# timoklein/alphazero-gym

Measured on AMD Instinct MI355X. Metric: MCTS sims/sec (whole node), Pendulum-v1 4096 trees n_sims=200, 1/2/4/8 GPU, higher is better.
Workload: dtype f32; 1 GPU; config C: Pendulum-v1 A0C, 4096 trees/GPU x 200 sims, 2x256 ELU policy/value MLP, c_uct=0.05 c_pw=1 kappa=0.5; trees_per_gpu=4096, n_sims=200, parallelism=1 GPU

## Files before the change

### alphazero_gym_amd/csrc/mlp.cuh

```cuda
#pragma once
#include "records.h"


typedef int i32x4 __attribute__((ext_vector_type(4)));


__device__ __forceinline__ f32x4 expm1f4_nonpos(f32x4 xc) {
    const f32x4 magic = {12582912.0f, 12582912.0f, 12582912.0f, 12582912.0f};
    const f32x4 l2e = {1.44269504088896341f, 1.44269504088896341f, 1.44269504088896341f, 1.44269504088896341f};
    const f32x4 ln2h = {0.693145751953125f, 0.693145751953125f, 0.693145751953125f, 0.693145751953125f};
    const f32x4 ln2l = {1.42860682030941723212e-6f, 1.42860682030941723212e-6f, 1.42860682030941723212e-6f, 1.42860682030941723212e-6f};
    const f32x4 kb = __builtin_elementwise_fma(xc, l2e, magic);
    const f32x4 kf = kb - magic;
    f32x4 r = __builtin_elementwise_fma(-kf, ln2h, xc);
    r = __builtin_elementwise_fma(-kf, ln2l, r);
    f32x4 p = {1.98412698412698413e-4f, 1.98412698412698413e-4f, 1.98412698412698413e-4f, 1.98412698412698413e-4f};
    const f32x4 c5 = {1.38888888888888894e-3f, 1.38888888888888894e-3f, 1.38888888888888894e-3f, 1.38888888888888894e-3f};
    const f32x4 c4 = {8.33333333333333322e-3f, 8.33333333333333322e-3f, 8.33333333333333322e-3f, 8.33333333333333322e-3f};
    const f32x4 c3 = {4.16666666666666644e-2f, 4.16666666666666644e-2f, 4.16666666666666644e-2f, 4.16666666666666644e-2f};
    const f32x4 c2 = {1.66666666666666657e-1f, 1.66666666666666657e-1f, 1.66666666666666657e-1f, 1.66666666666666657e-1f};
    const f32x4 half = {0.5f, 0.5f, 0.5f, 0.5f}, one = {1.0f, 1.0f, 1.0f, 1.0f};
    p = __builtin_elementwise_fma(p, r, c5);
    p = __builtin_elementwise_fma(p, r, c4);
    p = __builtin_elementwise_fma(p, r, c3);
    p = __builtin_elementwise_fma(p, r, c2);
    p = __builtin_elementwise_fma(p, r, half);
    f32x4 em1 = __builtin_elementwise_fma(p * r, r, r);
    const i32x4 scb = (((i32x4)kb) << 23) + 0x3F800000;
    const f32x4 sc = (f32x4)scb;
    return __builtin_elementwise_fma(sc, em1, sc - one);
}

template <bool RARE = true>
__device__ __forceinline__ f32x4 act4(int act, f32x4 v) {
    f32x4 pos;
    asm("v_max_f32 %0, 0, %1" : "=v"(pos.x) : "v"(v.x)); asm("v_max_f32 %0, 0, %1" : "=v"(pos.y) : "v"(v.y));
    asm("v_max_f32 %0, 0, %1" : "=v"(pos.z) : "v"(v.z)); asm("v_max_f32 %0, 0, %1" : "=v"(pos.w) : "v"(v.w));
    if (act == AZG_ACT_ELU) {
        f32x4 neg;
        neg.x = __builtin_amdgcn_fmed3f(v.x, -87.0f, 0.0f); neg.y = __builtin_amdgcn_fmed3f(v.y, -87.0f, 0.0f);
        neg.z = __builtin_amdgcn_fmed3f(v.z, -87.0f, 0.0f); neg.w = __builtin_amdgcn_fmed3f(v.w, -87.0f, 0.0f);
        return pos + expm1f4_nonpos(neg);
    }
    if (!RARE || act == AZG_ACT_RELU) return pos;
    f32x4 r;
    r.x = azg_activation(act, v.x); r.y = azg_activation(act, v.y); r.z = azg_activation(act, v.z); r.w = azg_activation(act, v.w);
    return r;
}

__device__ __forceinline__ f32x4 mfma4(f32x4 a, f32x4 b, f32x4 acc) {
    acc = __builtin_amdgcn_mfma_f32_16x16x4f32(a.x, b.x, acc, 0, 0, 0);
    acc = __builtin_amdgcn_mfma_f32_16x16x4f32(a.y, b.y, acc, 0, 0, 0);
    acc = __builtin_amdgcn_mfma_f32_16x16x4f32(a.z, b.z, acc, 0, 0, 0);
// ... 89 lines not shown
            } else {
#pragma unroll
                for (int i = 0; i < NT0; ++i) a0[i] = act4<false>(AZG_ACT_RELU, a0[i]);
            }
#pragma unroll
            for (int i = 0; i < NT0; ++i) actA[((wave - NW / 2) * NT0 + i) * 64 + lane] = a0[i];
            if (lane == 0) __hip_atomic_fetch_add(l0_flag, 1, __ATOMIC_RELEASE, __HIP_MEMORY_SCOPE_WORKGROUP);
        }
        const int want = (NW / 2) * step;
        while (__hip_atomic_load(l0_flag, __ATOMIC_ACQUIRE, __HIP_MEMORY_SCOPE_WORKGROUP) < want) __builtin_amdgcn_s_sleep(1);
    } else {
#pragma unroll
    for (int g = 0; g < NG; ++g) {
        float b;
        if constexpr (NT == 16) b = obsT[(lane >> 4) * (16 * NG) + g * 16 + (lane & 15)];
        else b = (lane & 15) < NT ? obsT[(lane >> 4) * (NT * NG) + g * NT + (lane & 15)] : 0.0f;
        float b2 = 0.0f;
        if constexpr (IN8) {
            if constexpr (NT == 16) b2 = obsT[(4 + (lane >> 4)) * (16 * NG) + g * 16 + (lane & 15)];
            else b2 = (lane & 15) < NT ? obsT[(4 + (lane >> 4)) * (NT * NG) + g * NT + (lane & 15)] : 0.0f;
        }
#pragma unroll
        for (int i = 0; i < NTW; ++i) {
            f32x4 a0;
            if constexpr (HP <= 256) {
                a0 = __builtin_amdgcn_mfma_f32_16x16x4f32(wr.w0[i], b, wr.b0[i], 0, 0, 0);
                if constexpr (IN8) { if (P.in8) a0 = __builtin_amdgcn_mfma_f32_16x16x4f32(wr.w0b[i], b2, a0, 0, 0, 0); }
            } else {
                const int nt = wave * NTW + i;
                a0 = __builtin_amdgcn_mfma_f32_16x16x4f32(P.W0[wofs + nt * 64 + lane], b, net_ptr(P.b0, wofs)[nt * 64 + lane], 0, 0, 0);
                if constexpr (IN8) { if (P.in8) a0 = __builtin_amdgcn_mfma_f32_16x16x4f32(P.W0b[wofs + nt * 64 + lane], b2, a0, 0, 0, 0); }
            }
            if constexpr (NREG == 0) h[g][i] = act4<true>(P.act, a0);
            else h[g][i] = a0;
        }
    }
    if constexpr (NREG > 0) {
        if (P.act == AZG_ACT_ELU) {
#pragma unroll
            for (int g = 0; g < NG; ++g)
#pragma unroll
                for (int i = 0; i < NTW; ++i) h[g][i] = act4<false>(AZG_ACT_ELU, h[g][i]);
        } else {
#pragma unroll
            for (int g = 0; g < NG; ++g)
#pragma unroll
                for (int i = 0; i < NTW; ++i) h[g][i] = act4<false>(AZG_ACT_RELU, h[g][i]);
        }
    }
    }
    if constexpr (NREG == 0) { if (P.layernorm) layer_norm_wg<HP>(P, 0, h[0], s_ln, wave, lane, wofs); }
    f32x4* buf = actA;
    f32x4* other = actB;
    if (NREG > 0) {
#pragma unroll
        for (int l = 0; l < NREG; ++l) {
            if (!(SPLIT && l == 0)) {
#pragma unroll
                for (int g = 0; g < NG; ++g)
#pragma unroll
                    for (int i = 0; i < NTW; ++i) buf[g * ABUF + (wave * NTW + i) * 64 + lane] = h[g][i];
                __syncthreads();
            }
            STAMP_M(m1, 4, 5);
            f32x4 acc[NG][NTW];
            f32x4 bcur[NG], bnext[NG];
#pragma unroll
            for (int g = 0; g < NG; ++g) {
#pragma unroll
                for (int i = 0; i < NTW; ++i) acc[g][i] = wr.b[l][i];
                bcur[g] = buf[g * ABUF + lane];
            }
#pragma unroll
            for (int s4 = 0; s4 < S4; ++s4) {
#pragma unroll
                for (int g = 0; g < NG; ++g) {
                    bnext[g] = bcur[g];
                    if (s4 + 1 < S4) bnext[g] = buf[g * ABUF + (s4 + 1) * 64 + lane];
                }
                __builtin_amdgcn_sched_barrier(0);
#pragma unroll
                for (int i = 0; i < NTW; ++i)
#pragma unroll
                    for (int g = 0; g < NG; ++g) acc[g][i] = __builtin_amdgcn_mfma_f32_16x16x4f32(wr.w[l][i][s4].x, bcur[g].x, acc[g][i], 0, 0, 0);
#pragma unroll
                for (int i = 0; i < NTW; ++i)
#pragma unroll
                    for (int g = 0; g < NG; ++g) acc[g][i] = __builtin_amdgcn_mfma_f32_16x16x4f32(wr.w[l][i][s4].y, bcur[g].y, acc[g][i], 0, 0, 0);
#pragma unroll
                for (int i = 0; i < NTW; ++i)
#pragma unroll
                    for (int g = 0; g < NG; ++g) acc[g][i] = __builtin_amdgcn_mfma_f32_16x16x4f32(wr.w[l][i][s4].z, bcur[g].z, acc[g][i], 0, 0, 0);
#pragma unroll
                for (int i = 0; i < NTW; ++i)
#pragma unroll
                    for (int g = 0; g < NG; ++g) acc[g][i] = __builtin_amdgcn_mfma_f32_16x16x4f32(wr.w[l][i][s4].w, bcur[g].w, acc[g][i], 0, 0, 0);
#pragma unroll
                for (int g = 0; g < NG; ++g) bcur[g] = bnext[g];
            }
            STAMP_M(m2, 5, 6);
            if (P.act == AZG_ACT_ELU) {
#pragma unroll
                for (int g = 0; g < NG; ++g)
#pragma unroll
                    for (int i = 0; i < NTW; ++i) h[g][i] = act4<false>(AZG_ACT_ELU, acc[g][i]);
            } else {
#pragma unroll
                for (int g = 0; g < NG; ++g)
#pragma unroll
                    for (int i = 0; i < NTW; ++i) h[g][i] = act4<false>(AZG_ACT_RELU, acc[g][i]);
            }
            STAMP_M(m2b, 6, -1);
            if (l == 0) { STAMP_M_ADD(4, m0, m1); }
            STAMP_M_ADD(5, m1, m2);
            STAMP_M_ADD(6, m2, m2b);
            f32x4* t = buf; buf = other; other = t;
        }
    } else {
        for (int l = 1; l < P.n_hidden; ++l) {
#pragma unroll
            for (int i = 0; i < NTW; ++i) buf[(wave * NTW + i) * 64 + lane] = h[0][i];
            __syncthreads();
            const f32x4* W = net_ptr(P.Wl[l - 1], wofs);
            const f32x4* bb = net_ptr(P.bl[l - 1], wofs);
            constexpr int TG = NTW < 4 ? NTW : 4;
#pragma unroll
            for (int tg = 0; tg < NTW; tg += TG) {
                f32x4 acc[TG];
#pragma unroll
                for (int i = 0; i < TG; ++i) acc[i] = bb[(wave * NTW + tg + i) * 64 + lane];
#pragma unroll 2
                for (int s4 = 0; s4 < S4; ++s4) {
                    f32x4 b = buf[s4 * 64 + lane];
                    f32x4 a[TG];
#pragma unroll
                    for (int i = 0; i < TG; ++i) a[i] = W[((wave * NTW + tg + i) * S4 + s4) * 64 + lane];
#pragma unroll
                    for (int i = 0; i < TG; ++i) acc[i] = __builtin_amdgcn_mfma_f32_16x16x4f32(a[i].x, b.x, acc[i], 0, 0, 0);
#pragma unroll
                    for (int i = 0; i < TG; ++i) acc[i] = __builtin_amdgcn_mfma_f32_16x16x4f32(a[i].y, b.y, acc[i], 0, 0, 0);
#pragma unroll
                    for (int i = 0; i < TG; ++i) acc[i] = __builtin_amdgcn_mfma_f32_16x16x4f32(a[i].z, b.z, acc[i], 0, 0, 0);
#pragma unroll
                    for (int i = 0; i < TG; ++i) acc[i] = __builtin_amdgcn_mfma_f32_16x16x4f32(a[i].w, b.w, acc[i], 0, 0, 0);
                }
#pragma unroll
                for (int i = 0; i < TG; ++i) h[0][tg + i] = act4<NREG == 0>(P.act, acc[i]);
            }
            if (P.layernorm) layer_norm_wg<HP>(P, l, h[0], s_ln, wave, lane, wofs);
            f32x4* t = buf; buf = other; other = t;
        }
    }
    {
        constexpr int NSUB = HP <= 256 ? 8 / NW : NTW / 4;
        constexpr int KS = 4 * NTW / NSUB;
        f32x4 acc[NG][NSUB];
#pragma unroll
        for (int g = 0; g < NG; ++g)
#pragma unroll
            for (int sc = 0; sc < NSUB; ++sc) acc[g][sc] = f32x4{0.0f, 0.0f, 0.0f, 0.0f};
#pragma unroll
        for (int j = 0; j < KS; ++j) {
#pragma unroll
            for (int sc = 0; sc < NSUB; ++sc) {
                const int ks = sc * KS + j, ti = ks >> 2, cmp = ks & 3;
                const f32x4 a = (NREG > 0) ? wr.wh[ti] : net_ptr(P.Whead, wofs)[(wave * NTW + ti) * 64 + lane];
#pragma unroll
                for (int g = 0; g < NG; ++g) acc[g][sc] = __builtin_amdgcn_mfma_f32_16x16x4f32(a[cmp], h[g][ti][cmp], acc[g][sc], 0, 0, 0);
            }
        }
#pragma unroll
        for (int g = 0; g < NG; ++g)
#pragma unroll
            for (int sc = 0; sc < NSUB; ++sc)
                if (PSTR == 64 || lane < 16) parts[(g * NCH + wave * NSUB + sc) * PSTR + lane] = acc[g][sc];
    }
    __syncthreads();
}

template <int NCH, int PSTR = 64>
__device__ __forceinline__ float head_output(const f32x4* parts, const float* s_bhead, int tl, int o) {
    float total = s_bhead[o];
    const int idx = (o >> 2) * 16 + tl;
#pragma unroll
    for (int w = 0; w < NCH; ++w) {
        f32x4 pv = parts[w * PSTR + idx];
        float p = (o & 3) == 0 ? pv.x : ((o & 3) == 1 ? pv.y : ((o & 3) == 2 ? pv.z : pv.w));
        total = total + p;
    }
    return total;
}

template <int NCH, int PSTR = 64>
__device__ __forceinline__ f32x4 head_output4(const f32x4* parts, const float* s_bhead, int tl) {
    f32x4 total = {s_bhead[0], s_bhead[1], s_bhead[2], s_bhead[3]};
#pragma unroll
    for (int w = 0; w < NCH; ++w) {
        const f32x4 pv = parts[w * PSTR + tl];
        total.x = total.x + pv.x; total.y = total.y + pv.y; total.z = total.z + pv.z; total.w = total.w + pv.w;
    }
    return total;
}

#define GMM_MAXC 5
template <int NCH, int PSTR = 64>
__device__ __forceinline__ void gmm_params(const f32x4* parts, const float* s_bhead, int tl, int C, float ls_min, float ls_max, float* d) {
    float mx = head_output<NCH, PSTR>(parts, s_bhead, tl, 1 + 2 * C);
#pragma unroll
    for (int c = 1; c < GMM_MAXC; ++c)
        if (c < C) { float v = head_output<NCH, PSTR>(parts, s_bhead, tl, 1 + 2 * C + c); mx = v > mx ? v : mx; }
    float ex[GMM_MAXC], sum = 0.0f, cum = 0.0f;
#pragma unroll
    for (int c = 0; c < GMM_MAXC; ++c) {
        ex[c] = 0.0f;
        if (c < C) { ex[c] = azg_expf(head_output<NCH, PSTR>(parts, s_bhead, tl, 1 + 2 * C + c) - mx); sum = sum + ex[c]; }
    }
#pragma unroll
    for (int c = 0; c < GMM_MAXC; ++c) {
        d[c] = 0.0f; d[GMM_MAXC + c] = 0.0f; d[2 * GMM_MAXC + c] = 2.0f;
        if (c < C) {
            float ls = head_output<NCH, PSTR>(parts, s_bhead, tl, 1 + C + c);
            ls = ls < ls_min ? ls_min : (ls > ls_max ? ls_max : ls);
            d[c] = head_output<NCH, PSTR>(parts, s_bhead, tl, 1 + c);
            d[GMM_MAXC + c] = azg_expf(ls);
            cum = cum + ex[c] / sum;
            d[2 * GMM_MAXC + c] = cum;
        }
    }
}

__device__ __forceinline__ void gmm_pick(const float* d, int C, unsigned long long seed, unsigned gtree, unsigned search, unsigned k,
                                         float* mu, float* sg) {
    azg_u32x4 b = azg_draw(seed, gtree, search, k, AZG_STREAM_PW);
    float u = azg_u01(b.v[2]);
    float m = 0.0f, s = 0.0f;
    bool found = false;
#pragma unroll
    for (int i = 0; i < GMM_MAXC; ++i) {
        bool last = (i == C - 1);
        if (i < C && !found && (u < d[2 * GMM_MAXC + i] || last)) { m = d[i]; s = d[GMM_MAXC + i]; found = true; }
    }
    *mu = m;
// ... 3 lines not shown
```

### alphazero_gym_amd/csrc/search_kernel.cuh

```cuda
#pragma once
#include "records.h"
#include "env.cuh"
#include "mlp.cuh"
#include "tree.cuh"
#include "tree_phases.cuh"
#include "results.cuh"
#ifndef AZG_DEFER
#define AZG_DEFER 1
#endif

struct LdsLayout {
    size_t act_off;
    size_t tree_off;
    size_t per_tree;
    size_t state_off;
    size_t total;
};
__host__ __device__ inline LdsLayout lds_layout(int tab_n, int n_sims, int HP, int NG, int nbuf, int R, bool cont, int tlds, int lds_state = 0, int NT = 16) {
    LdsLayout L;
    L.act_off = ((size_t)tab_n * 8 + (size_t)(n_sims + 2) * 2 + 15) / 16 * 16;
    L.tree_off = L.act_off + (size_t)nbuf * NG * HP * 64;
    L.per_tree = (size_t)R * 16 + (cont ? (size_t)POOL_UNITS(R) * (tlds == TS_LDS9 ? 8 : 4) : (size_t)R * 4);
    L.per_tree = (L.per_tree + 15) / 16 * 16;
    L.state_off = 0;
// ... 64 lines not shown
        constexpr int S4 = HP / 16;
#pragma unroll
        for (int l = 0; l < NREG; ++l) {
#pragma unroll
            for (int i = 0; i < NTW; ++i) {
                wr.b[l][i] = net_ptr(P.bl[l], wofs)[(wave * NTW + i) * 64 + lane];
#pragma unroll
                for (int s4 = 0; s4 < S4; ++s4) wr.w[l][i][s4] = net_ptr(P.Wl[l], wofs)[((wave * NTW + i) * S4 + s4) * 64 + lane];
            }
        }
#pragma unroll
        for (int i = 0; i < NTW; ++i) wr.wh[i] = net_ptr(P.Whead, wofs)[(wave * NTW + i) * 64 + lane];
    }

    struct Ctx {
        int sub, tl, tree; bool has_tree, live; unsigned gtree; size_t tb;
        Cold* cold; double* edge_W; float* action; TreeStore<TLDS> ts; const f32x4* my_parts;
    };
    auto make_ctx = [&](int t) {
        Ctx c;
        const int w = t >> 6, ln = t & 63;
        c.sub = ln & 15;
        c.has_tree = w < NWALK && (ln >> 4) < TPV;
        c.tl = c.has_tree ? w * TPV + (ln >> 4) : 0;
        c.tree = tree0 + c.tl;
        c.live = c.has_tree && c.tl < n_live;
        c.gtree = (unsigned)(P.tree_base + c.tree);
        c.tb = (size_t)(c.live ? c.tree : 0) * P.R;
        c.cold = P.cold + c.tb;
        c.edge_W = P.edge_W + c.tb;
        c.action = P.action + c.tb;
        if constexpr (TLDS != TS_GLOBAL) {
            char* base = (char*)s_dyn + L.tree_off + L.per_tree * c.tl;
            c.ts.hot = (Rec*)base;
            c.ts.pool = (typename TreeStore<TLDS>::PoolId*)(base + (size_t)P.R * 16);
            c.ts.prior = (float*)(base + (size_t)P.R * 16);
            c.ts.state = L.state_off ? (double*)(base + L.state_off) : nullptr;
        } else {
            c.ts.hot = (Rec*)(P.hot + c.tb);
            c.ts.child = P.child + c.tb * P.Kp;
            c.ts.prior = P.prior + c.tb;
        }
        c.my_parts = s_parts + (c.tl / NT) * NCH * PSTR;
        return c;
    };
    Ctx cx = make_ctx(tid);

#ifdef AZG_STAMPS
    unsigned long long st_acc[16] = {0, 0, 0, 0, 0, 0, 0, 0, 0, 0, 0, 0, 0, 0, 0, 0};
#endif
    TreeState st = {};
    st.need_eval = false;
    BDeferred bdef = {};
    if (cx.has_tree) tree_init_root<ENV, TLDS, TPW, IN8>(P, st, cx.ts, cx.cold, cx.edge_W, cx.action, cx.tree, cx.live, cx.sub, cx.tl, cx.gtree, s_obsT);
    __syncthreads();

    constexpr bool MULTI = !CONT;
    static_assert(!(LEAN && MULTI), "discrete 8-wave shapes: extend the LEAN packing first");
    int my_sim = -1;
    for (int sim = -1; sim < P.n_sims; ++sim) {
        STAMP2(t_a, 0, -1);
        __syncthreads();
        if constexpr (MULTI) { if (*(volatile int*)&s_done >= n_live) break; }
        STAMP2(t_b, 0, 1);
        if constexpr (DEFER) {
            STAMP2(t_b2a, 12, -1);
            if (cx.live) tree_phase_b2<ENV, TLDS, SPEC>(P, st, cx.ts, cx.cold, cx.edge_W, cx.action, bdef, cx.sub, cx.gtree, s_pw);
            bdef.pending = false;
            STAMP2(t_b2b, 12, -1);
#ifdef AZG_STAMP_ONLY
            STAMP_ADD(12, t_b2a, t_b2b);
#endif
        }
        unsigned pk0 = 0, pk1 = 0, pk2 = 0, pk3 = 0;
        int tid_o = tid;
        if constexpr (LEAN) {
            pk0 = (unsigned)st.nrec | ((unsigned)st.leaf << 16);
            pk1 = (unsigned)st.path_D | ((unsigned)st.kbase << 16);
            pk2 = (unsigned)(st.my_depth + 1) | ((unsigned)st.pid << 16);
            pk3 = (unsigned)st.ptop | ((unsigned)st.need_eval << 16) | ((unsigned)st.resume << 20);
            asm volatile("" : "+v"(pk0), "+v"(pk1), "+v"(pk2), "+v"(pk3));
        }
#ifdef AZG_STAMPS
        mlp_forward<HP, NREG, NW, NG, PSTR, WR, NT, IN8, DEFER>(P, wr, s_obsT, s_actA, s_actB, s_parts, s_ln, wave, lane, st_acc, &s_l0, sim + 2, wofs);
#else
        mlp_forward<HP, NREG, NW, NG, PSTR, WR, NT, IN8, DEFER>(P, wr, s_obsT, s_actA, s_actB, s_parts, s_ln, wave, lane, &s_l0, sim + 2, wofs);
#endif
        STAMP2(t_c, 1, 2);
        if constexpr (LEAN) {
            asm volatile("" : "+v"(pk0), "+v"(pk1), "+v"(pk2), "+v"(pk3), "+v"(tid_o));
            st.nrec = (int)(pk0 & 0xffffu); st.leaf = (int)(pk0 >> 16);
            st.path_D = (int)(pk1 & 0xffffu); st.kbase = (int)(pk1 >> 16);
            st.my_depth = (int)(pk2 & 0xffffu) - 1; st.pid = (int)(pk2 >> 16);
            st.ptop = (int)(pk3 & 0xffffu); st.need_eval = ((pk3 >> 16) & 1u) != 0; st.resume = (int)(pk3 >> 20);
            cx = make_ctx(tid_o);
            st.pr = 0.0; st.pW = 0.0;
            if (cx.live && (MULTI ? my_sim : sim) >= 0 && st.my_depth >= 1) {
                st.pr = CONT ? cx.cold[st.pid].r : discrete_env_reward(Spec<SPEC, ENV>::env(P));
                st.pW = cx.edge_W[st.pid];
            }
        }
        if constexpr (!MULTI) {
            if (cx.live) tree_phase_a<ENV, TLDS, GMM, NCH, PSTR, !CONT, SPEC>(P, st, cx.ts, cx.cold, cx.edge_W, cx.action, cx.tb, sim, cx.sub, cx.tl % NT, cx.gtree, cx.my_parts, s_bhead, s_sqrt STAMP_ARG, s_pw);
            if (sim == P.n_sims - 1) break;
            if constexpr (DEFER) { if (sim < 0 && cx.live) eps_prepare(P, st, cx.gtree, cx.sub); }
            tree_fence();
            STAMP2(t_d, 2, 3);
            st.need_eval = false;
            if (cx.live) tree_phase_b<ENV, TLDS, GMM, TPW, unsigned short, !LEAN, !CONT, SPEC, IN8, DEFER>(P, st, cx.ts, cx.cold, cx.edge_W, cx.action, cx.tb, cx.sub, cx.tl, cx.gtree, s_sqrt, s_pw, s_obsT STAMP_ARG, &bdef);
            tree_fence();
            STAMP2(t_e, 3, -1);
            STAMP_ADD(2, t_c, t_d);
            STAMP_ADD(3, t_d, t_e);
        } else {
            bool run = cx.live && my_sim < P.n_sims;
            int k = 0;
            while (run) {
                STAMP2(t_c2, 2, -1);
                tree_phase_a<ENV, TLDS, GMM, NCH, PSTR, !CONT, SPEC>(P, st, cx.ts, cx.cold, cx.edge_W, cx.action, cx.tb, my_sim, cx.sub, cx.tl % NT, cx.gtree, cx.my_parts, s_bhead, s_sqrt STAMP_ARG, s_pw);
                tree_fence();
                STAMP2(t_d, 2, 3);
                st.need_eval = false;
                if (my_sim == P.n_sims - 1) {
                    my_sim = P.n_sims;
                    if (cx.sub == 0) atomicAdd(&s_done, 1);
                    run = false;
                } else {
                    my_sim += 1;
                    tree_phase_b<ENV, TLDS, GMM, TPW, unsigned short, !LEAN, !CONT, SPEC, IN8>(P, st, cx.ts, cx.cold, cx.edge_W, cx.action, cx.tb, cx.sub, cx.tl, cx.gtree, s_sqrt, s_pw, s_obsT STAMP_ARG);
                    tree_fence();
                    k += 1;
                    if (st.need_eval || k >= P.trace_cap) run = false;
                }
                STAMP2(t_e, 3, -1);
                STAMP_ADD(2, t_c2, t_d);
                STAMP_ADD(3, t_d, t_e);
            }
        }
        STAMP_ADD(0, t_a, t_b);
        STAMP_ADD(1, t_b, t_c);
    }
    const int nrec = st.nrec;
    const int sub = cx.sub, tree = cx.tree;
    const bool live = cx.live;
    const size_t tb = cx.tb;
    const TreeStore<TLDS>& ts = cx.ts;
#ifdef AZG_STAMPS
    if (lane == 0) for (int i = 0; i < 16; ++i) P.stamps[((size_t)blockIdx.x * NW + wave) * 16 + i] = st_acc[i];
#endif
    if (live) results_for_tree<CONT, TLDS>(P, ts, cx.cold, cx.action, tb, tree, sub);
    if (live) {
        if (sub == 0) P.n_rec[tree] = nrec;
        if constexpr (TLDS != TS_GLOBAL) {
            if (P.publish) {
                RecL* gh = P.hot + tb;
                for (int j = sub; j < nrec; j += 16) {
                    Rec h = ts.hot[j];
                    RecL o;
                    o.Q = h.Q; o.edge_n = h.edge_n; o.node_n = h.node_n; o.parent = (short)h.parent; o.n_child = h.n_child;
                    o.first = CONT ? 0 : h.first; o.flags = h.flags; o.pad = 0;
                    gh[j] = o;
                    if (CONT) {
// ... 10 lines not shown
```

### alphazero_gym_amd/csrc/tree.cuh

```cuda
#pragma once
#include "records.h"

__device__ __forceinline__ void tree_fence() { __builtin_amdgcn_fence(__ATOMIC_ACQ_REL, "wavefront"); }

__device__ __forceinline__ double tree_div(double n, double d) {
    double r = __builtin_amdgcn_rcp(d);
    double e = __builtin_fma(-d, r, 1.0);
    r = __builtin_fma(r, e, r);
    e = __builtin_fma(-d, r, 1.0);
    r = __builtin_fma(r, e, r);
    double q = n * r;
    double rem = __builtin_fma(-d, q, n);
    return __builtin_fma(rem, r, q);
}


template <int CTRL>
__device__ __forceinline__ int dpp_i32(int v) { return __builtin_amdgcn_update_dpp(0, v, CTRL, 0xf, 0xf, false); }
template <int CTRL>
__device__ __forceinline__ double dpp_f64(double v) {
    unsigned long long u = azg_d2u(v);
    unsigned lo = (unsigned)dpp_i32<CTRL>((int)(unsigned)u), hi = (unsigned)dpp_i32<CTRL>((int)(unsigned)(u >> 32));
    return azg_u2d(((unsigned long long)hi << 32) | lo);
}
template <int CTRL>
__device__ __forceinline__ float dpp_f32(float v) { return __builtin_bit_cast(float, dpp_i32<CTRL>(__builtin_bit_cast(int, v))); }
#define DPP_QUAD_BCAST1 0x55
#define DPP_QUAD_XOR1 0xB1
#define DPP_QUAD_XOR2 0x4E
#define DPP_ROW_ROR4 0x124
#define DPP_ROW_ROR8 0x128
#define DPP_ROW_ROR15 0x12F

__device__ __forceinline__ double rowmax16(double u, bool valid) {
    double m = valid ? u : -__builtin_huge_val();
    double o;
    o = dpp_f64<DPP_QUAD_XOR1>(m); m = o > m ? o : m;
    o = dpp_f64<DPP_QUAD_XOR2>(m); m = o > m ? o : m;
    o = dpp_f64<DPP_ROW_ROR4>(m); m = o > m ? o : m;
    o = dpp_f64<DPP_ROW_ROR8>(m); m = o > m ? o : m;
    return m;
}
__device__ __forceinline__ int rowmin16(int c) {
    int t;
    t = dpp_i32<DPP_QUAD_XOR1>(c); c = t < c ? t : c;
    t = dpp_i32<DPP_QUAD_XOR2>(c); c = t < c ? t : c;
    t = dpp_i32<DPP_ROW_ROR4>(c); c = t < c ? t : c;
    t = dpp_i32<DPP_ROW_ROR8>(c); c = t < c ? t : c;
    return c;
}
__device__ __forceinline__ int argmax16(double u, bool valid, int sub) {
    double m = rowmax16(u, valid);
    return rowmin16((valid && u == m) ? sub : 99);
}
__device__ __forceinline__ int rowmax16_i32(int v) {
    int o;
    o = dpp_i32<DPP_QUAD_XOR1>(v); v = o > v ? o : v;
    o = dpp_i32<DPP_QUAD_XOR2>(v); v = o > v ? o : v;
    o = dpp_i32<DPP_ROW_ROR4>(v); v = o > v ? o : v;
    o = dpp_i32<DPP_ROW_ROR8>(v); v = o > v ? o : v;
    return v;
}
__device__ __forceinline__ unsigned rowmax16_u32(unsigned v) {
    unsigned o;
    o = (unsigned)dpp_i32<DPP_QUAD_XOR1>((int)v); v = o > v ? o : v;
    o = (unsigned)dpp_i32<DPP_QUAD_XOR2>((int)v); v = o > v ? o : v;
    o = (unsigned)dpp_i32<DPP_ROW_ROR4>((int)v); v = o > v ? o : v;
    o = (unsigned)dpp_i32<DPP_ROW_ROR8>((int)v); v = o > v ? o : v;
    return v;
}
__device__ __forceinline__ int argmax16_payload(double u, bool valid, int sub, int payload) {
    const long long bits = (long long)azg_d2u(u);
    const long long key = bits ^ ((bits >> 63) & 0x7fffffffffffffffLL);
    const int hi = valid ? (int)(key >> 32) : (int)0x80000000;
    const unsigned lo = (unsigned)key;
    const int mh = rowmax16_i32(hi);
    const bool top = valid && hi == mh;
    const unsigned ml = rowmax16_u32(top ? lo : 0u);
    return rowmin16((top && lo == ml) ? ((sub << 16) | payload) : 0x7fffffff) & 0xffff;
}

#define DPP_QUAD_BCAST0 0x00
__device__ __forceinline__ int argmax2_payload(double u, int sub, int payload) {
    const double o = dpp_f64<DPP_QUAD_XOR1>(u);
    const int po = dpp_i32<DPP_QUAD_XOR1>(payload);
// ... 206 lines not shown
```

### alphazero_gym_amd/csrc/tree_phases.cuh

```cuda
#pragma once
#ifndef EARLY_COLD
#define EARLY_COLD 1
#endif
#include "records.h"
#include "env.cuh"
#include "mlp.cuh"
#include "tree.cuh"

struct TreeState {
    int nrec;
    unsigned eps_draws;
    int leaf;
    bool need_eval;
    int path_D;
    int my_depth, pid;
    double pr, pW;
    int kbase;
    float eps_c;
    float eps_next;
    int ptop;
    int resume;
    double chainR;
    bool repeat;
};
// ... 117 lines not shown
    const double U1 = h1.Q + (double)pc1 * tree_div(sq, (double)((int)h1.edge_n + 1));
    const int win = c0 + (U0 >= U1 ? 0 : 1);
    if (mine) set_best<false>(&ts.hot[p], hp, win);
    return win;
}

template <int ENV, int TLDS, int TPW = 16, bool OBS8 = false>
__device__ __forceinline__ void tree_init_root(const KParams& P, TreeState& st, const TreeStore<TLDS>& ts, Cold* cold, double* edge_W,
                                               float* action, int tree, bool live, int sub, int tl, unsigned gtree, float* obsT) {
    constexpr bool CONT = EnvFamily<ENV>::CONT;
    constexpr int S = CONT ? 2 : 4;
    typedef typename TreeStore<TLDS>::Rec Rec;
    st.nrec = 1; st.eps_draws = 0; st.leaf = 0; st.need_eval = live;
    st.path_D = 0; st.my_depth = -1; st.pid = 0; st.pr = 0.0; st.pW = 0.0;
    st.kbase = 1; st.eps_c = 0.0f; st.eps_next = 0.0f; st.ptop = 0; st.resume = 0; st.chainR = 0.0; st.repeat = false;
    if (CONT && live) st.eps_c = azg_normal(P.seed, gtree, P.search_idx, (unsigned)(st.kbase + sub));
        double rs[S], sn;
#pragma unroll
        for (int k = 0; k < S; ++k) rs[k] = (live && k < P.S) ? P.roots[(size_t)tree * P.S + k] : 0.0;
        float obs[OBS8 ? 8 : 4];
        if constexpr (OBS8) { sn = 0.0; azg_acrobot_obs(rs, obs); obs[6] = 0.0f; obs[7] = 0.0f; }
        else env_obs<ENV == AZG_ENV_ACROBOT ? AZG_ENV_CARTPOLE : ENV>(rs, obs, &sn);
        if (live && sub == 0) {
            Rec h = make_edge<Rec>(0.0, 0);
            h.node_n = (decltype(h.node_n))P.carry[tree];
            h.flags = FLAG_EXPANDED;
            clear_pad(h);
            if (CONT) set_wnext(h, pw_at(P.pw_need, (int)P.carry[tree], P.n_sims + 1) > 0);
            ts.hot[0] = h;
            Cold c;
#pragma unroll
            for (int k = 0; k < 4; ++k) c.s[k] = k < S ? rs[k] : 0.0;
            if (CONT) c.s[2] = sn;
            c.r = 0.0; c.V = 0.0f; c.mu = 0.0f; c.sg = 0.0f; c.pad = 0.0f;
            cold[0] = c;
            edge_W[0] = 0.0;
            if (CONT) action[0] = 0.0f;
            if constexpr (!CONT && TLDS != TS_GLOBAL) {
                if (ts.state) {
#pragma unroll
                    for (int k = 0; k < 4; ++k) ts.state[k] = rs[k];
                }
            }
        }
        if constexpr (!OBS8) {
            if (sub < 4) obsT[sub * TPW + tl] = live ? obs[sub] : 0.0f;
        } else if (sub < 8) {
            float v = sub == 0 ? obs[0] : (sub == 1 ? obs[1] : (sub == 2 ? obs[2] : obs[3]));
            if (sub >= 4) v = sub == 4 ? obs[4] : (sub == 5 ? obs[5] : (sub == 6 ? obs[6] : obs[7]));
            obsT[sub * TPW + tl] = live ? v : 0.0f;
        }
}

template <int ENV, int TLDS, bool GMM, int NCH, int PSTR = 64, bool RESUME = false, int SPEC = 0, typename PW = int>
__device__ __forceinline__ void tree_phase_a(const KParams& P, TreeState& st, const TreeStore<TLDS>& ts, Cold* cold, double* edge_W,
                                             float* action, size_t tb, int sim, int sub, int tl, unsigned gtree, const f32x4* parts,
                                             const float* bhead, const double* s_sqrt STAMP_PARAM_OPT, const PW* s_pw = nullptr) {
    constexpr bool CONT = EnvFamily<ENV>::CONT;
    typedef typename TreeStore<TLDS>::Rec Rec;
    float V = 0.0f;
    STAMP_A(ta0, 4, -1);
    if (st.need_eval) {
        f32x4 out4 = {0.0f, 0.0f, 0.0f, 0.0f};
        if constexpr (!CONT) { out4 = head_output4<NCH, PSTR>(parts, bhead, tl); V = out4.x; }
        else V = head_output<NCH, PSTR>(parts, bhead, tl, 0);
        if (CONT) {
            float mu, sg;
            float gd[15];
            if constexpr (GMM) {
                gmm_params<NCH, PSTR>(parts, bhead, tl, P.ncomp, P.ls_min, P.ls_max, gd);
                mu = gd[0]; sg = gd[GMM_MAXC];
                float* g = P.gmm + (tb + st.leaf) * 3 * GMM_MAXC;
                if (sub == 0) {
#pragma unroll
                    for (int i = 0; i < 3 * GMM_MAXC; ++i) g[i] = gd[i];
                }
            } else {
                mu = head_output<NCH, PSTR>(parts, bhead, tl, 1);
                float ls = head_output<NCH, PSTR>(parts, bhead, tl, 2);
                ls = ls < P.ls_min ? P.ls_min : (ls > P.ls_max ? P.ls_max : ls);
                sg = azg_expf(ls);
            }
            if (sub == 0) { cold[st.leaf].V = V; cold[st.leaf].mu = mu; cold[st.leaf].sg = sg; }
            if (sim < 0) {
                int k = st.nrec++;
                if constexpr (GMM) gmm_pick(gd, P.ncomp, P.seed, gtree, P.search_idx, (unsigned)k, &mu, &sg);
                float eps = __shfl(st.eps_c, k - st.kbase, 16);
                float a = P.bound_f * azg_tanhf(mu + sg * eps);
                if (sub == 0) {
                    Rec h = make_edge<Rec>((double)V, 0);
                    clear_pad(h);
                    ts.hot[k] = h;
                    edge_W[k] = 0.0;
                    action[k] = a;
                }
                ts.child_append(0, make_edge<Rec>(0.0, 0), 0, k, st.ptop, sub == 0, P.Kp,
                                pw_at(P.pw_need, (int)ts.hot[0].node_n, P.n_sims + 1) - 1 > 0);
            }
        } else {
            const int A = Spec<SPEC, ENV>::A(P);
            float my_logit = sub == 0 ? out4.y : (sub == 1 ? out4.z : out4.w);
            if (A > 3 && sub >= 3 && sub < A) my_logit = head_output<NCH, PSTR>(parts, bhead, tl, 1 + sub);
            float mx = out4.y;
            if (A == 2) {
                mx = out4.z > mx ? out4.z : mx;
            } else {
                for (int a = 1; a < A; ++a) { const float v = __shfl(my_logit, a, 16); mx = v > mx ? v : mx; }
            }
            const float e_mine = azg_expf(my_logit - mx);
            float sum;
            if (A == 2) {
                sum = dpp_f32<DPP_QUAD_BCAST0>(e_mine) + dpp_f32<DPP_QUAD_BCAST1>(e_mine);
            } else {
                sum = 0.0f;
                for (int a = 0; a < A; ++a) sum = sum + __shfl(e_mine, a, 16);
            }
            int k0 = st.nrec;
            st.nrec += A;
            if (sub < A) {
                float prior_a = e_mine / sum;
                Rec h = make_edge<Rec>((double)V, st.leaf);
                clear_pad(h);
                ts.hot[k0 + sub] = h;
                ts.prior[k0 + sub] = prior_a;
                edge_W[k0 + sub] = 0.0;
            }
            if (sub == 0) {
                cold[st.leaf].V = V;
                ts.hot[st.leaf].n_child = (decltype(ts.hot[st.leaf].n_child))A;
                ts.hot[st.leaf].first = (decltype(ts.hot[st.leaf].first))k0;
            }
            if (Spec<SPEC, ENV>::plain(P)) {
                if (A == 2) {
                    const int nn = (int)ts.hot[st.leaf].node_n;
                    double sq;
                    if (Spec<SPEC, ENV>::in_table(P, nn)) sq = s_sqrt[nn];
// ... 54 lines not shown
        st.eps_c = azg_normal(P.seed, gtree, P.search_idx, (unsigned)(st.kbase + sub));
    }
    st.eps_next = __shfl(st.eps_c, st.nrec - st.kbase, 16);
}

struct BDeferred {
    bool pending, widen;
    int p, chosen;
    float cact;
};

template <int ENV, int TLDS, int SPEC, bool FETCH = false, typename PW = int>
__device__ __forceinline__ void tree_phase_b2(const KParams& P, TreeState& st, const TreeStore<TLDS>& ts, Cold* cold, double* edge_W, float* action,
                                              const BDeferred& d, int sub, unsigned gtree, const PW* s_pw) {
    typedef typename TreeStore<TLDS>::Rec Rec;
    static_assert(ENV == AZG_ENV_PENDULUM_V1, "deferred expansion: the Pendulum family");
    if (!d.pending) return;
    const double ps0 = cold[d.p].s[0], ps1 = cold[d.p].s[1];
    if (d.widen) {
        const float V = cold[d.p].V;
        const Rec hp = ts.hot[d.p];
        if (sub == 0) {
            Rec h = make_edge<Rec>((double)V, d.p);
            h.flags = FLAG_EXPANDED;
            clear_pad(h);
            set_wnext(h, P.pw0 > 0);
            ts.hot[d.chosen] = h;
            edge_W[d.chosen] = 0.0;
            action[d.chosen] = d.cact;
        }
        ts.child_append(d.p, hp, (int)hp.n_child, d.chosen, st.ptop, sub == 0, P.Kp,
                        pw_at(s_pw, (int)hp.node_n, P.n_sims + 1) - ((int)hp.n_child + 1) > 0);
    } else if (sub == 0) {
        Rec h = ts.hot[d.chosen];
        h.flags = FLAG_EXPANDED;
        set_wnext(h, P.pw0 > 0);
        ts.hot[d.chosen] = h;
    }
    const double sp[2] = {ps0, ps1};
    const double r = pendulum_reward(sp, d.cact) / P.reward_scale;
    if constexpr (FETCH) { if (sub == (st.path_D & 15)) st.pr = r; }
    if (sub == 0) {
        float zero = 0.0f;
        asm volatile("" : "+v"(zero));
        Cold* c = cold + d.chosen;
        c->s[3] = 0.0; c->r = r; c->V = zero; c->mu = zero; c->sg = zero; c->pad = zero;
    }
    eps_prepare(P, st, gtree, sub);
}

template <int ENV, int TLDS, bool GMM, int TPW = 16, typename PW = int, bool FETCH = true, bool RESUME = false, int SPEC = 0, bool OBS8 = false, bool DEFER = false>
__device__ __forceinline__ void tree_phase_b(const KParams& P, TreeState& st, const TreeStore<TLDS>& ts, Cold* cold, double* edge_W,
                                             float* action, size_t tb, int sub, int tl, unsigned gtree, const double* s_sqrt,
                                             const PW* s_pw, float* obsT STAMP_PARAM, BDeferred* def = nullptr) {
    static_assert(!DEFER || (ENV == AZG_ENV_PENDULUM_V1 && !GMM), "deferred expansion: Pendulum family, squashed-Normal head");
    constexpr bool CONT = EnvFamily<ENV>::CONT;
    constexpr int S = CONT ? 2 : 4;
    typedef typename TreeStore<TLDS>::Rec Rec;
    st.need_eval = false;
    if (CONT && !DEFER && st.nrec >= st.kbase + 16) {
        st.kbase = st.nrec;
        st.eps_c = azg_normal(P.seed, gtree, P.search_idx, (unsigned)(st.kbase + sub));
    }
    int p = 0;
    bool resumed = false;
    st.repeat = false;
    if constexpr (RESUME && !CONT) {
        if (Spec<SPEC, ENV>::plain(P) && Spec<SPEC, ENV>::A(P) == 2 && st.resume > 0) {
            resumed = true;
            p = __shfl(st.pid, st.resume, 16);
            if (st.my_depth > st.resume) st.my_depth = -1;
            st.path_D = st.resume;
        }
    }
    const double r_step = CONT ? 0.0 : discrete_env_reward(Spec<SPEC, ENV>::env(P));
    const bool keep_slot = !CONT && FETCH && resumed && st.my_depth >= 1;
    Rec hp = ts.hot[p];
    Cold cp;
    bool from_cold = true;
    if constexpr (!CONT && TLDS != TS_GLOBAL) from_cold = (ts.state == nullptr);
    if (from_cold) cp = cold[p];
    else { cp.s[0] = cp.s[1] = cp.s[2] = cp.s[3] = 0.0; }
    if (!resumed) { st.path_D = 0; st.my_depth = sub == 0 ? 0 : -1; st.pid = 0; }
    if (!keep_slot) { st.pr = 0.0; st.pW = 0.0; }
    int chosen = 0;
    bool widen = false, hit_terminal = false;
    if constexpr (RESUME && !CONT) {
        hit_terminal = resumed && (hp.flags & FLAG_TERMINAL);
        st.repeat = FETCH && hit_terminal;
    }
    STAMP2(tb0, 13, -1);
    while (!hit_terminal) {
        STAMP3(tl0, 7, 8, 11);
        const int K = hp.n_child;
        if (CONT) {
            widen = get_wnext(hp);
            if (widen) break;
        }
        if (CONT || !Spec<SPEC, ENV>::plain(P)) {
            int pick = -1;
            if (!Spec<SPEC, ENV>::eps0(P)) {
                azg_u32x4 b = azg_draw(P.seed, gtree, P.search_idx, st.eps_draws++, AZG_STREAM_EPS);
                if ((double)azg_u01(b.v[0]) < P.epsilon) pick = (int)(b.v[1] % (unsigned)K);
            }
            chosen = select_child<ENV, TLDS, Rec, SPEC>(P, ts, p, hp, sub, s_sqrt, pick, gtree);
        } else {
            chosen = rec_best<CONT>(hp);
        }
        STAMP2(tl1, 7, -1);
        STAMP_ADD(7, tl0, tl1);
        STAMP2(tl2, 8, 9);
        Cold cn;
        if constexpr (CONT && EARLY_COLD) cn = cold[chosen];
        Rec hc = ts.hot[chosen];
        if (!(hc.flags & FLAG_EXPANDED)) break;
        STAMP2(tl3, 9, 10);
        st.path_D += 1;
        p = chosen;
        hp = hc;
        if (sub == (st.path_D & 15)) {
            st.my_depth = st.path_D; st.pid = chosen;
            if (CONT && FETCH) { st.pr = EARLY_COLD ? cn.r : cold[chosen].r; st.pW = edge_W[chosen]; }
            if (!CONT && FETCH) { st.pr = r_step; st.pW = edge_W[chosen]; }
        }
        if constexpr (EnvFamily<ENV>::TERM) {
            if (hc.flags & FLAG_TERMINAL) { hit_terminal = true; break; }
        }
        if (CONT) { if constexpr (EARLY_COLD) cp = cn; else cp = cold[p]; }
        else if (from_cold) { cp.s[0] = cold[p].s[0]; cp.s[1] = cold[p].s[1]; cp.s[2] = cold[p].s[2]; cp.s[3] = cold[p].s[3]; }
        STAMP2(tl4, 10, 11);
        STAMP_ADD(8, tl0, tl2);
        STAMP_ADD(9, tl2, tl3);
        STAMP_ADD(10, tl3, tl4);
        STAMP_ADD(11, tl0, tl4);
#if defined(AZG_STAMPS) && !defined(AZG_STAMP_ONLY)
// ... 104 lines not shown
```

Baseline: 548.4 million sims/s.

## Interleave head MFMAs with final activation and defer leaf head stores

For the 8-wave, 2-tile register MLP configuration, the value/policy head matmul is folded into the last hidden layer's activation, using sched_group_barriers to interleave MFMAs with the ELU VALU work, so the separate head loop is skipped. In phase A on the continuous, non-GMM deferred path, each lane reads one head output and broadcasts V via DPP. The mu/log-sigma writes to the cold leaf record are postponed to a LateHead that is flushed at the start of phase B, or after the last simulation, which takes work off the critical path. This adds scheduling constraints and spreads the cold writes across lanes. Correctness depends on the leaf index and the pending flag staying consistent between phases.

Result: slower. 531.9 million sims/s (-3.0%).

```diff
diff --git a/alphazero_gym_amd/csrc/mlp.cuh b/alphazero_gym_amd/csrc/mlp.cuh
--- a/alphazero_gym_amd/csrc/mlp.cuh
+++ b/alphazero_gym_amd/csrc/mlp.cuh
@@ -1,4 +1,5 @@
 #pragma once
+#include <type_traits>
 #include "records.h"
 
 
@@ -194,6 +195,8 @@
     if constexpr (NREG == 0) { if (P.layernorm) layer_norm_wg<HP>(P, 0, h[0], s_ln, wave, lane, wofs); }
     f32x4* buf = actA;
     f32x4* other = actB;
+    constexpr bool HEADMIX = NREG > 0 && NG == 1 && NW == 8 && NTW == 2 && HP <= 256;
+    [[maybe_unused]] f32x4 hacc = {0.0f, 0.0f, 0.0f, 0.0f};
     if (NREG > 0) {
 #pragma unroll
         for (int l = 0; l < NREG; ++l) {
@@ -241,7 +244,23 @@
                 for (int g = 0; g < NG; ++g) bcur[g] = bnext[g];
             }
             STAMP_M(m2, 5, 6);
-            if (P.act == AZG_ACT_ELU) {
+            bool mixed = false;
+            if constexpr (HEADMIX) { if (l == NREG - 1) {
+                mixed = true;
+                auto mix = [&](auto ACT) {
+                    h[0][0] = act4<false>(decltype(ACT)::value, acc[0][0]);
+                    __builtin_amdgcn_sched_barrier(0);
+                    h[0][1] = act4<false>(decltype(ACT)::value, acc[0][1]);
+                    hacc = mfma4(wr.wh[0], h[0][0], hacc);
+#pragma unroll
+                    for (int q = 0; q < 4; ++q) { __builtin_amdgcn_sched_group_barrier(0x008, 1, 0); __builtin_amdgcn_sched_group_barrier(0x002, 10, 0); }
+                    __builtin_amdgcn_sched_barrier(0);
+                    hacc = mfma4(wr.wh[1], h[0][1], hacc);
+                };
+                if (P.act == AZG_ACT_ELU) mix(std::integral_constant<int, AZG_ACT_ELU>()); else mix(std::integral_constant<int, AZG_ACT_RELU>());
+            } }
+            if (mixed) {
+            } else if (P.act == AZG_ACT_ELU) {
 #pragma unroll
                 for (int g = 0; g < NG; ++g)
 #pragma unroll
@@ -302,7 +321,7 @@
 #pragma unroll
             for (int sc = 0; sc < NSUB; ++sc) acc[g][sc] = f32x4{0.0f, 0.0f, 0.0f, 0.0f};
 #pragma unroll
-        for (int j = 0; j < KS; ++j) {
+        for (int j = 0; j < (HEADMIX ? 0 : KS); ++j) {
 #pragma unroll
             for (int sc = 0; sc < NSUB; ++sc) {
                 const int ks = sc * KS + j, ti = ks >> 2, cmp = ks & 3;
@@ -315,7 +334,7 @@
         for (int g = 0; g < NG; ++g)
 #pragma unroll
             for (int sc = 0; sc < NSUB; ++sc)
-                if (PSTR == 64 || lane < 16) parts[(g * NCH + wave * NSUB + sc) * PSTR + lane] = acc[g][sc];
+                if (PSTR == 64 || lane < 16) parts[(g * NCH + wave * NSUB + sc) * PSTR + lane] = HEADMIX ? hacc : acc[g][sc];
     }
     __syncthreads();
 }
@@ -330,6 +349,15 @@
         float p = (o & 3) == 0 ? pv.x : ((o & 3) == 1 ? pv.y : ((o & 3) == 2 ? pv.z : pv.w));
         total = total + p;
     }
+    return total;
+}
+
+template <int NCH, int PSTR = 64>
+__device__ __forceinline__ float head_output_lane(const f32x4* parts, const float* s_bhead, int tl, int o) {
+    const float* pf = (const float*)(parts + tl) + o;
+    float total = s_bhead[o];
+#pragma unroll
+    for (int w = 0; w < NCH; ++w) total = total + pf[w * PSTR * 4];
     return total;
 }
 
diff --git a/alphazero_gym_amd/csrc/search_kernel.cuh b/alphazero_gym_amd/csrc/search_kernel.cuh
--- a/alphazero_gym_amd/csrc/search_kernel.cuh
+++ b/alphazero_gym_amd/csrc/search_kernel.cuh
@@ -140,6 +140,8 @@
     TreeState st = {};
     st.need_eval = false;
     BDeferred bdef = {};
+    LateHead late = {};
+    LateHead* const latep = DEFER ? &late : nullptr;
     if (cx.has_tree) tree_init_root<ENV, TLDS, TPW, IN8>(P, st, cx.ts, cx.cold, cx.edge_W, cx.action, cx.tree, cx.live, cx.sub, cx.tl, cx.gtree, s_obsT);
     __syncthreads();
 
@@ -189,13 +191,16 @@
             }
         }
         if constexpr (!MULTI) {
-            if (cx.live) tree_phase_a<ENV, TLDS, GMM, NCH, PSTR, !CONT, SPEC>(P, st, cx.ts, cx.cold, cx.edge_W, cx.action, cx.tb, sim, cx.sub, cx.tl % NT, cx.gtree, cx.my_parts, s_bhead, s_sqrt STAMP_ARG, s_pw);
-            if (sim == P.n_sims - 1) break;
+            if (cx.live) tree_phase_a<ENV, TLDS, GMM, NCH, PSTR, !CONT, SPEC>(P, st, cx.ts, cx.cold, cx.edge_W, cx.action, cx.tb, sim, cx.sub, cx.tl % NT, cx.gtree, cx.my_parts, s_bhead, s_sqrt STAMP_ARG, s_pw, latep);
+            if (sim == P.n_sims - 1) {
+                if constexpr (DEFER) { if (cx.live) late_head_store(P, cx.cold, st.leaf, late, cx.sub); }
+                break;
+            }
             if constexpr (DEFER) { if (sim < 0 && cx.live) eps_prepare(P, st, cx.gtree, cx.sub); }
             tree_fence();
             STAMP2(t_d, 2, 3);
             st.need_eval = false;
-            if (cx.live) tree_phase_b<ENV, TLDS, GMM, TPW, unsigned short, !LEAN, !CONT, SPEC, IN8, DEFER>(P, st, cx.ts, cx.cold, cx.edge_W, cx.action, cx.tb, cx.sub, cx.tl, cx.gtree, s_sqrt, s_pw, s_obsT STAMP_ARG, &bdef);
+            if (cx.live) tree_phase_b<ENV, TLDS, GMM, TPW, unsigned short, !LEAN, !CONT, SPEC, IN8, DEFER>(P, st, cx.ts, cx.cold, cx.edge_W, cx.action, cx.tb, cx.sub, cx.tl, cx.gtree, s_sqrt, s_pw, s_obsT STAMP_ARG, &bdef, latep);
             tree_fence();
             STAMP2(t_e, 3, -1);
             STAMP_ADD(2, t_c, t_d);
diff --git a/alphazero_gym_amd/csrc/tree.cuh b/alphazero_gym_amd/csrc/tree.cuh
--- a/alphazero_gym_amd/csrc/tree.cuh
+++ b/alphazero_gym_amd/csrc/tree.cuh
@@ -31,6 +31,7 @@
 #define DPP_ROW_ROR4 0x124
 #define DPP_ROW_ROR8 0x128
 #define DPP_ROW_ROR15 0x12F
+#define DPP_ROW_SHARE0 0x150
 
 __device__ __forceinline__ double rowmax16(double u, bool valid) {
     double m = valid ? u : -__builtin_huge_val();
diff --git a/alphazero_gym_amd/csrc/tree_phases.cuh b/alphazero_gym_amd/csrc/tree_phases.cuh
--- a/alphazero_gym_amd/csrc/tree_phases.cuh
+++ b/alphazero_gym_amd/csrc/tree_phases.cuh
@@ -193,17 +193,34 @@
         }
 }
 
+__device__ __forceinline__ float normal_sigma(const KParams& P, float ls) {
+    ls = ls < P.ls_min ? P.ls_min : (ls > P.ls_max ? P.ls_max : ls);
+    return azg_expf(ls);
+}
+
+struct LateHead { float val; bool pending; };
+__device__ __forceinline__ void late_head_store(const KParams& P, Cold* cold, int leaf, LateHead& lh, int sub) {
+    const float sg = normal_sigma(P, lh.val);
+    float* f = &cold[leaf].V;
+    if (lh.pending && sub < 3) f[sub] = sub == 2 ? sg : lh.val;
+    lh.pending = false;
+}
+
 template <int ENV, int TLDS, bool GMM, int NCH, int PSTR = 64, bool RESUME = false, int SPEC = 0, typename PW = int>
 __device__ __forceinline__ void tree_phase_a(const KParams& P, TreeState& st, const TreeStore<TLDS>& ts, Cold* cold, double* edge_W,
                                              float* action, size_t tb, int sim, int sub, int tl, unsigned gtree, const f32x4* parts,
-                                             const float* bhead, const double* s_sqrt STAMP_PARAM_OPT, const PW* s_pw = nullptr) {
+                                             const float* bhead, const double* s_sqrt STAMP_PARAM_OPT, const PW* s_pw = nullptr,
+                                             LateHead* late = nullptr) {
     constexpr bool CONT = EnvFamily<ENV>::CONT;
     typedef typename TreeStore<TLDS>::Rec Rec;
     float V = 0.0f;
     STAMP_A(ta0, 4, -1);
     if (st.need_eval) {
         f32x4 out4 = {0.0f, 0.0f, 0.0f, 0.0f};
+        float own = 0.0f;
+        const bool lane_form = CONT && !GMM && late != nullptr;
         if constexpr (!CONT) { out4 = head_output4<NCH, PSTR>(parts, bhead, tl); V = out4.x; }
+        else if (lane_form) { own = head_output_lane<NCH, PSTR>(parts, bhead, tl, sub < 2 ? sub : 2); V = dpp_f32<DPP_ROW_SHARE0>(own); }
         else V = head_output<NCH, PSTR>(parts, bhead, tl, 0);
         if (CONT) {
             float mu, sg;
@@ -216,13 +233,15 @@
 #pragma unroll
                     for (int i = 0; i < 3 * GMM_MAXC; ++i) g[i] = gd[i];
                 }
+            } else if (lane_form && sim >= 0) {
+                late->val = own; late->pending = true;
+                mu = 0.0f; sg = 0.0f;
             } else {
-                mu = head_output<NCH, PSTR>(parts, bhead, tl, 1);
-                float ls = head_output<NCH, PSTR>(parts, bhead, tl, 2);
-                ls = ls < P.ls_min ? P.ls_min : (ls > P.ls_max ? P.ls_max : ls);
-                sg = azg_expf(ls);
-            }
-            if (sub == 0) { cold[st.leaf].V = V; cold[st.leaf].mu = mu; cold[st.leaf].sg = sg; }
+                if (lane_form) { mu = __shfl(own, 1, 16); sg = __shfl(own, 2, 16); }
+                else { mu = head_output<NCH, PSTR>(parts, bhead, tl, 1); sg = head_output<NCH, PSTR>(parts, bhead, tl, 2); }
+                sg = normal_sigma(P, sg);
+            }
+            if (!(lane_form && sim >= 0)) { if (sub == 0) { cold[st.leaf].V = V; cold[st.leaf].mu = mu; cold[st.leaf].sg = sg; } }
             if (sim < 0) {
                 int k = st.nrec++;
                 if constexpr (GMM) gmm_pick(gd, P.ncomp, P.seed, gtree, P.search_idx, (unsigned)k, &mu, &sg);
@@ -383,7 +402,7 @@
 template <int ENV, int TLDS, bool GMM, int TPW = 16, typename PW = int, bool FETCH = true, bool RESUME = false, int SPEC = 0, bool OBS8 = false, bool DEFER = false>
 __device__ __forceinline__ void tree_phase_b(const KParams& P, TreeState& st, const TreeStore<TLDS>& ts, Cold* cold, double* edge_W,
                                              float* action, size_t tb, int sub, int tl, unsigned gtree, const double* s_sqrt,
-                                             const PW* s_pw, float* obsT STAMP_PARAM, BDeferred* def = nullptr) {
+                                             const PW* s_pw, float* obsT STAMP_PARAM, BDeferred* def = nullptr, LateHead* late = nullptr) {
     static_assert(!DEFER || (ENV == AZG_ENV_PENDULUM_V1 && !GMM), "deferred expansion: Pendulum family, squashed-Normal head");
     constexpr bool CONT = EnvFamily<ENV>::CONT;
     constexpr int S = CONT ? 2 : 4;
@@ -412,6 +431,7 @@
     if constexpr (!CONT && TLDS != TS_GLOBAL) from_cold = (ts.state == nullptr);
     if (from_cold) cp = cold[p];
     else { cp.s[0] = cp.s[1] = cp.s[2] = cp.s[3] = 0.0; }
+    if constexpr (CONT && !GMM) { if (late) late_head_store(P, cold, st.leaf, *late, sub); }
     if (!resumed) { st.path_D = 0; st.my_depth = sub == 0 ? 0 : -1; st.pid = 0; }
     if (!keep_slot) { st.pr = 0.0; st.pW = 0.0; }
     int chosen = 0;
```
